# haoyu94/RoITr

Hardware: AMD Instinct MI355X
Metric: point-cloud pairs/s (higher is better)
Workload: dtype f32

## Files before the change

roitr_amd/csrc/local_block.hip:

```cpp
#include "common.h"
#include "prof.h"
#include "roitr_engine.h"
#include <mutex>
#include <vector>

namespace {

typedef float f32x4 __attribute__((ext_vector_type(4)));
typedef float f32x16 __attribute__((ext_vector_type(16)));
typedef float f32x2 __attribute__((ext_vector_type(2)));
typedef __bf16 bf16x8 __attribute__((ext_vector_type(8)));
typedef __bf16 bf16x2 __attribute__((ext_vector_type(2)));


template <int CTRL> __device__ __forceinline__ float dpp_mov(float v)
{
    return __int_as_float(__builtin_amdgcn_update_dpp(0, __float_as_int(v), CTRL, 0xf, 0xf, true));
}
template <int HL> __device__ __forceinline__ float head_allsum(float v)
{
    v += dpp_mov<0xB1>(v);
    v += dpp_mov<0x4E>(v);
    if (HL == 8) v += dpp_mov<0x141>(v);
    return v;
}

struct Acc { f32x4 t[2][2]; };

__device__ __forceinline__ void acc_zero(Acc& a)
{
#pragma unroll
    for (int m = 0; m < 2; ++m)
#pragma unroll
        for (int n = 0; n < 2; ++n) a.t[m][n] = f32x4{0.f, 0.f, 0.f, 0.f};
}

template <int H, int AP, int RT = 1, bool FR = false, bool APF = false>
__device__ __forceinline__ void gemm_phase(Acc (&acc)[RT], const float* __restrict__ A, int Ka, const float* __restrict__ W, int ldw, int k_w0,
                                           int r0, int c0, int tid)
{
    const int lane = tid & 63, i = lane & 15, g = lane >> 4;
    const float* wl = FR ? W + ((size_t)(c0 >> 5) * (ldw >> 5) + (k_w0 >> 5)) * 1024 + 4 * lane : W + (size_t)(c0 + i) * ldw + k_w0 + 4 * g;
    const int os = FR ? 1024 : 32, oc = FR ? 512 : 16, on = FR ? 256 : 16 * ldw;
    const float* al = A + (r0 + i) * AP + 4 * g;
    float4 bn[2][2];
#pragma unroll
    for (int c = 0; c < 2; ++c) { bn[c][0] = *reinterpret_cast<const float4*>(wl + c * oc); bn[c][1] = *reinterpret_cast<const float4*>(wl + c * oc + on); }
    float4 an0, an1;
    if (APF) { an0 = *reinterpret_cast<const float4*>(al); an1 = *reinterpret_cast<const float4*>(al + 16 * AP); }
    for (int k0 = 0; k0 < Ka; k0 += 32) {
        float4 bc[2][2];
#pragma unroll
        for (int c = 0; c < 2; ++c) { bc[c][0] = bn[c][0]; bc[c][1] = bn[c][1]; }
        if (k0 + 32 < Ka) {
            const float* wn = wl + (size_t)((k0 >> 5) + 1) * os;
#pragma unroll
            for (int c = 0; c < 2; ++c) {
                bn[c][0] = *reinterpret_cast<const float4*>(wn + c * oc);
                bn[c][1] = *reinterpret_cast<const float4*>(wn + c * oc + on);
            }
        }
#pragma unroll
        for (int c = 0; c < 2; ++c) {
            const float4 b0 = bc[c][0], b1 = bc[c][1];
#pragma unroll
            for (int t = 0; t < RT; ++t) {
                float4 a0, a1;
                if (APF) {
                    a0 = an0; a1 = an1;
                    const bool last = t + 1 == RT && c == 1;
                    const int tn = t + 1 < RT ? t + 1 : 0, kn = last ? k0 + 32 : k0 + (t + 1 < RT ? 16 * c : 16);
                    if (!last || k0 + 32 < Ka) {
                        an0 = *reinterpret_cast<const float4*>(al + 32 * tn * AP + kn);
                        an1 = *reinterpret_cast<const float4*>(al + (32 * tn + 16) * AP + kn);
                    }
                    __builtin_amdgcn_sched_barrier(0);
                } else {
                    a0 = *reinterpret_cast<const float4*>(al + 32 * t * AP + k0 + 16 * c);
                    a1 = *reinterpret_cast<const float4*>(al + (32 * t + 16) * AP + k0 + 16 * c);
                }
#define LB_STEP(S)                                                                                                  \
                acc[t].t[0][0] = __builtin_amdgcn_mfma_f32_16x16x4f32(a0.S, b0.S, acc[t].t[0][0], 0, 0, 0);          \
                acc[t].t[0][1] = __builtin_amdgcn_mfma_f32_16x16x4f32(a0.S, b1.S, acc[t].t[0][1], 0, 0, 0);          \
                acc[t].t[1][0] = __builtin_amdgcn_mfma_f32_16x16x4f32(a1.S, b0.S, acc[t].t[1][0], 0, 0, 0);          \
                acc[t].t[1][1] = __builtin_amdgcn_mfma_f32_16x16x4f32(a1.S, b1.S, acc[t].t[1][1], 0, 0, 0)
                LB_STEP(x); LB_STEP(y); LB_STEP(z); LB_STEP(w);
#undef LB_STEP
            }
        }
    }
}
template <int H, int AP, bool FR = false, bool APF = false>
__device__ __forceinline__ void gemm_phase1(Acc& acc, const float* __restrict__ A, int Ka, const float* __restrict__ W, int ldw, int k_w0,
                                           int r0, int c0, int tid)
{
    gemm_phase<H, AP, 1, FR, APF>(reinterpret_cast<Acc (&)[1]>(acc), A, Ka, W, ldw, k_w0, r0, c0, tid);
}

template <int DP>
__device__ __forceinline__ void acc_store(const Acc& acc, const float* __restrict__ bias, float* __restrict__ D, int r0, int c0, int lane)
{
#pragma unroll
    for (int n = 0; n < 2; ++n) {
        const int col = c0 + 16 * n + (lane & 15);
        const float bv = bias[col];
#pragma unroll
        for (int m = 0; m < 2; ++m)
#pragma unroll
            for (int r = 0; r < 4; ++r) D[(r0 + 16 * m + 4 * (lane >> 4) + r) * DP + col] = acc.t[m][n][r] + bv;
    }
}

__device__ __forceinline__ unsigned lb_pack_bf16(float x, float y)
{
    f32x2 v = {x, y};
    return __builtin_bit_cast(unsigned, __builtin_convertvector(v, bf16x2));
}
template <int AP, int RT>
__device__ __forceinline__ void gemm_phase_bf16(f32x16 (&acc)[RT], const float* __restrict__ A, int Ka, const unsigned short* __restrict__ Wb, int ldw,
                                                int k_w0, int r0, int c0, int tid)
{
    const int lane = tid & 63, ml = lane & 31, kh = lane >> 5;
    const unsigned short* w = Wb + (size_t)(c0 + ml) * ldw + k_w0 + 8 * kh;
    uint4 bn[2];
    bn[0] = *reinterpret_cast<const uint4*>(w); bn[1] = *reinterpret_cast<const uint4*>(w + 16);
    for (int k0 = 0; k0 < Ka; k0 += 32) {
        uint4 bc[2] = {bn[0], bn[1]};
        if (k0 + 32 < Ka) { bn[0] = *reinterpret_cast<const uint4*>(w + k0 + 32); bn[1] = *reinterpret_cast<const uint4*>(w + k0 + 48); }
#pragma unroll
        for (int c = 0; c < 2; ++c) {
            const bf16x8 b = __builtin_bit_cast(bf16x8, bc[c]);
#pragma unroll
            for (int t = 0; t < RT; ++t) {
                const float* ap = A + (r0 + 32 * t + ml) * AP + k0 + 16 * c + 8 * kh;
                const float4 x0 = *reinterpret_cast<const float4*>(ap), x1 = *reinterpret_cast<const float4*>(ap + 4);
                const uint4 h = make_uint4(lb_pack_bf16(x0.x, x0.y), lb_pack_bf16(x0.z, x0.w), lb_pack_bf16(x1.x, x1.y), lb_pack_bf16(x1.z, x1.w));
                acc[t] = __builtin_amdgcn_mfma_f32_32x32x16_bf16(__builtin_bit_cast(bf16x8, h), b, acc[t], 0, 0, 0);
            }
        }
    }
}
template <int DP>
__device__ __forceinline__ void acc_store32(const f32x16& acc, const float* __restrict__ bias, float* __restrict__ D, int r0, int c0, int lane)
{
    const int col = c0 + (lane & 31);
    const float bv = bias[col];
#pragma unroll
    for (int i = 0; i < 16; ++i) D[(r0 + (i & 3) + 8 * (i >> 2) + 4 * (lane >> 5)) * DP + col] = acc[i] + bv;
}
template <bool MB, int RT> struct RegionAcc { Acc a[RT]; };
template <int RT> struct RegionAcc<true, RT> { f32x16 a[RT]; };
template <bool MB, int RT> __device__ __forceinline__ void region_zero(RegionAcc<MB, RT>& r)
{
#pragma unroll
    for (int t = 0; t < RT; ++t) {
        if constexpr (MB) {
#pragma unroll
            for (int i = 0; i < 16; ++i) r.a[t][i] = 0.f;
        } else acc_zero(r.a[t]);
    }
}
template <bool MB, int H, int AP, int RT, bool FR, bool APF>
__device__ __forceinline__ void region_gemm(RegionAcc<MB, RT>& r, const float* __restrict__ A, int Ka, const float* __restrict__ W,
                                            const unsigned short* __restrict__ Wb, int ldw, int k_w0, int r0, int c0, int tid)
{
    if constexpr (MB) gemm_phase_bf16<AP, RT>(r.a, A, Ka, Wb, ldw, k_w0, r0, c0, tid);
    else gemm_phase<H, AP, RT, FR, APF>(r.a, A, Ka, W, ldw, k_w0, r0, c0, tid);
}
template <bool MB, int DP, int RT>
__device__ __forceinline__ void region_store(const RegionAcc<MB, RT>& r, const float* __restrict__ bias, float* __restrict__ D, int r0, int c0, int lane)
{
#pragma unroll
    for (int t = 0; t < RT; ++t) {
        if constexpr (MB) acc_store32<DP>(r.a[t], bias, D, r0 + 32 * t, c0, lane);
        else acc_store<DP>(r.a[t], bias, D, r0 + 32 * t, c0, lane);
    }
}

template <bool KVH>
__device__ __forceinline__ float4 ld_kv4(const float* kv, size_t row, int ld, int col)
{
    if (KVH) {
        const uint2 t = *reinterpret_cast<const uint2*>(reinterpret_cast<const unsigned short*>(kv) + row * ld + col);
        return make_float4(__uint_as_float(t.x << 16), __uint_as_float(t.x & 0xffff0000u), __uint_as_float(t.y << 16), __uint_as_float(t.y & 0xffff0000u));
    }
    return *reinterpret_cast<const float4*>(kv + row * ld + col);
}

template <int H, int K, int TM, int DBG = 0, bool KVH = false, bool MB = false, bool FR = false>
__global__ __launch_bounds__(256, (K <= 8 && TM * H <= 4096) ? 3 : 2) void local_block_kernel(RoitrLocalBlock a)
{
    constexpr int AP = H + 4;
    constexpr int LPN = H / 4;
    constexpr int NPW = 64 / LPN;
    constexpr int HL = LPN / 4;
    constexpr int HV = H / 64;
    __shared__ __attribute__((aligned(16))) float R1[TM * AP];
    __shared__ __attribute__((aligned(16))) float R2[TM * AP];
    __shared__ int ids[TM];
    int tid = threadIdx.x, lane = tid & 63, wave = tid >> 6;
    const int ntiles = (a.M + TM - 1) / TM;
    const int tile = xcd_block_id(ntiles);
    if (tile >= ntiles) return;
    const int s0 = tile * TM;
    if (tid < TM) {
        const int sl = s0 + tid < a.M ? s0 + tid : s0;
        ids[tid] = a.node_order ? __float_as_int(reinterpret_cast<const float4*>(a.node_order)[sl].w) : sl;
    }
    __syncthreads();
    {
        constexpr int F4 = H / 4;
        constexpr int NX = TM * F4 / 256;
        float4 xr[NX];
#pragma unroll
        for (int u = 0; u < NX; ++u) {
            const int e = tid + 256 * u;
            xr[u] = *reinterpret_cast<const float4*>(a.x + (size_t)ids[e / F4] * H + 4 * (e % F4));
        }
#pragma unroll
        for (int u = 0; u < NX; ++u) {
            const int e = tid + 256 * u;
            *reinterpret_cast<float4*>(R1 + (e / F4) * AP + 4 * (e % F4)) = xr[u];
        }
    }
    constexpr int NC = H / 32, RT = TM * H / (32 * 32 * 4);
    constexpr bool APF = H == 128 && RT == 2;
    int r0 = (wave / NC) * 32 * RT;
    int c0 = (wave % NC) * 32;
    RegionAcc<MB, RT> acc;
    auto zero_all = [&]() { region_zero<MB, RT>(acc); };
    auto store_all = [&](const float* bias) { region_store<MB, AP, RT>(acc, bias, R2, r0, c0, lane); };
    __syncthreads();
    zero_all();
    if (DBG != 2) region_gemm<MB, H, AP, RT, FR, APF>(acc, R1, H, a.wq, a.wq_h, H, 0, r0, c0, tid);
    store_all(a.bq);
    __syncthreads();
    if (DBG != 1) {
        const int ns = lane / LPN, j = lane % LPN, jq = j % HL;
        const int t4 = jq & 3;
        constexpr int NRD = TM / (4 * NPW);
        int gi[K]; float pv[K];
        auto load_ids = [&](int rd_, int (&g_)[K], float (&p_)[K]) {
            const int node_ = ids[(rd_ * 4 + wave) * NPW + ns];
            const int4* gp = reinterpret_cast<const int4*>(a.group_idx + (size_t)node_ * K);
#pragma unroll
            for (int q4 = 0; q4 < K / 4; ++q4) { const int4 t = gp[q4]; g_[4 * q4] = t.x; g_[4 * q4 + 1] = t.y; g_[4 * q4 + 2] = t.z; g_[4 * q4 + 3] = t.w; }
            const float* pf = a.ppf + (size_t)node_ * K * 4 + t4;
#pragma unroll
            for (int kk = 0; kk < K; ++kk) p_[kk] = pf[kk * 4];
        };
        load_ids(0, gi, pv);
        for (int rd = 0; rd < NRD; ++rd) {
            const int row = (rd * 4 + wave) * NPW + ns;
            constexpr bool V_EARLY = K <= 8;
            float4 kr[K], vr[K];
#pragma unroll
            for (int kk = 0; kk < K; ++kk) kr[kk] = ld_kv4<KVH>(a.kv, (size_t)gi[kk], 2 * H, 4 * j);
            if (V_EARLY) {
#pragma unroll
                for (int kk = 0; kk < K; ++kk) vr[kk] = ld_kv4<KVH>(a.kv, (size_t)gi[kk], 2 * H, H + 4 * j);
            }
            int gn[K]; float pn[K];
            if (rd + 1 < NRD) load_ids(rd + 1, gn, pn);
            float4 wpe4[4]; float bpe4[4];
#pragma unroll
            for (int i = 0; i < 4; ++i) { wpe4[i] = reinterpret_cast<const float4*>(a.wpe)[4 * j + i]; bpe4[i] = a.bpe[4 * j + i]; }
            float4 qv = *reinterpret_cast<const float4*>(R2 + row * AP + 4 * j);
            float ec, c4;
            {
                float p0 = 0.f, p1 = 0.f, p2 = 0.f, p3 = 0.f, p4 = 0.f;
                const float qs[4] = {qv.x, qv.y, qv.z, qv.w};
#pragma unroll
                for (int i = 0; i < 4; ++i) {
                    p0 = fmaf(wpe4[i].x, qs[i], p0); p1 = fmaf(wpe4[i].y, qs[i], p1); p2 = fmaf(wpe4[i].z, qs[i], p2);
                    p3 = fmaf(wpe4[i].w, qs[i], p3); p4 = fmaf(bpe4[i], qs[i], p4);
                }
                p0 = head_allsum<HL>(p0); p1 = head_allsum<HL>(p1); p2 = head_allsum<HL>(p2); p3 = head_allsum<HL>(p3); p4 = head_allsum<HL>(p4);
                ec = jq < 4 ? (jq == 0 ? p0 : (jq == 1 ? p1 : (jq == 2 ? p2 : p3))) * a.scale : 0.f;
                c4 = jq == 0 ? p4 * a.scale : 0.f;
            }
            qv.x *= a.scale; qv.y *= a.scale; qv.z *= a.scale; qv.w *= a.scale;
            float sc[K];
            float mx = -INFINITY;
#pragma unroll
            for (int kk = 0; kk < K; ++kk) {
                float d = fmaf(ec, pv[kk], c4);
                d = fmaf(qv.x, kr[kk].x, d); d = fmaf(qv.y, kr[kk].y, d); d = fmaf(qv.z, kr[kk].z, d); d = fmaf(qv.w, kr[kk].w, d);
                d = head_allsum<HL>(d);
                sc[kk] = d;
                mx = fmaxf(mx, d);
            }
            if (!V_EARLY) {
#pragma unroll
                for (int kk = 0; kk < K; ++kk) vr[kk] = ld_kv4<KVH>(a.kv, (size_t)gi[kk], 2 * H, H + 4 * j);
            }
            float sum = 0.f;
#pragma unroll
            for (int kk = 0; kk < K; ++kk) { sc[kk] = __expf(sc[kk] - mx); sum += sc[kk]; }
            float pb = 0.f;
            float4 o = make_float4(0.f, 0.f, 0.f, 0.f);
            const float inv = 1.0f / sum;
#pragma unroll
            for (int kk = 0; kk < K; ++kk) {
                const float p = sc[kk] * inv;
                pb = fmaf(p, pv[kk], pb);
                o.x = fmaf(p, vr[kk].x, o.x); o.y = fmaf(p, vr[kk].y, o.y); o.z = fmaf(p, vr[kk].z, o.z); o.w = fmaf(p, vr[kk].w, o.w);
            }
            const float b0 = dpp_mov<0x00>(pb), b1 = dpp_mov<0x55>(pb), b2 = dpp_mov<0xAA>(pb), b3 = dpp_mov<0xFF>(pb);
            const float4 bias = *reinterpret_cast<const float4*>(a.bvpe + 4 * j);
            const float4 w0 = reinterpret_cast<const float4*>(a.wvpe)[4 * j], w1 = reinterpret_cast<const float4*>(a.wvpe)[4 * j + 1];
            const float4 w2 = reinterpret_cast<const float4*>(a.wvpe)[4 * j + 2], w3 = reinterpret_cast<const float4*>(a.wvpe)[4 * j + 3];
            o.x += w0.x * b0 + w0.y * b1 + w0.z * b2 + w0.w * b3 + bias.x;
            o.y += w1.x * b0 + w1.y * b1 + w1.z * b2 + w1.w * b3 + bias.y;
            o.z += w2.x * b0 + w2.y * b1 + w2.z * b2 + w2.w * b3 + bias.z;
            o.w += w3.x * b0 + w3.y * b1 + w3.z * b2 + w3.w * b3 + bias.w;
            *reinterpret_cast<float4*>(R2 + row * AP + 4 * j) = o;
            if (rd + 1 < NRD) {
#pragma unroll
                for (int kk = 0; kk < K; ++kk) { gi[kk] = gn[kk]; pv[kk] = pn[kk]; }
            }
        }
    }
    {
        int t2 = tid;
        asm volatile("" : "+v"(t2));
        tid = t2; lane = t2 & 63; wave = t2 >> 6;
        r0 = (wave / NC) * 32 * RT; c0 = (wave % NC) * 32;
    }
    __syncthreads();
    zero_all();
    if (DBG != 2) {
    region_gemm<MB, H, AP, RT, FR, APF>(acc, R2, H, a.wcat, a.wcat_h, 2 * H, 0, r0, c0, tid);
    region_gemm<MB, H, AP, RT, FR, APF>(acc, R1, H, a.wcat, a.wcat_h, 2 * H, H, r0, c0, tid);
    }
    __syncthreads();
    store_all(a.bcat);
    __syncthreads();
    {
        const int lr = lane >> 4, lc = lane & 15;
        float4 gam[HV], bet[HV];
#pragma unroll
        for (int i = 0; i < HV; ++i) { gam[i] = reinterpret_cast<const float4*>(a.norm_w)[lc + 16 * i]; bet[i] = reinterpret_cast<const float4*>(a.norm_b)[lc + 16 * i]; }
#pragma unroll
        for (int u = 0; u < TM / 16; ++u) {
            const int rl = (u * 4 + wave) * 4 + lr;
            float4 t[HV];
            float s_ = 0.f;
#pragma unroll
            for (int i = 0; i < HV; ++i) { t[i] = *reinterpret_cast<const float4*>(R2 + rl * AP + 4 * (lc + 16 * i)); s_ += (t[i].x + t[i].y) + (t[i].z + t[i].w); }
            const float mean = row_allsum(s_) / (float)H;
            float q_ = 0.f;
#pragma unroll
            for (int i = 0; i < HV; ++i) {
                const float dx = t[i].x - mean, dy = t[i].y - mean, dz = t[i].z - mean, dw = t[i].w - mean;
                q_ += (dx * dx + dy * dy) + (dz * dz + dw * dw);
            }
            const float rstd = 1.0f / sqrtf(row_allsum(q_) / (float)H + a.eps);
#pragma unroll
            for (int i = 0; i < HV; ++i) {
                float4 y;
                y.x = (t[i].x - mean) * rstd * gam[i].x + bet[i].x; y.y = (t[i].y - mean) * rstd * gam[i].y + bet[i].y;
                y.z = (t[i].z - mean) * rstd * gam[i].z + bet[i].z; y.w = (t[i].w - mean) * rstd * gam[i].w + bet[i].w;
                *reinterpret_cast<float4*>(R1 + rl * AP + 4 * (lc + 16 * i)) = y;
            }
        }
    }
    float4 xres[TM / 16][HV];
    {
        const int lr = lane >> 4, lc = lane & 15;
#pragma unroll
        for (int u = 0; u < TM / 16; ++u) {
            const size_t node = (size_t)ids[(u * 4 + wave) * 4 + lr];
#pragma unroll
            for (int i = 0; i < HV; ++i) xres[u][i] = *reinterpret_cast<const float4*>(a.x + node * H + 4 * (lc + 16 * i));
        }
    }
    __syncthreads();
    zero_all();
    if (DBG != 2) region_gemm<MB, H, AP, RT, FR, APF>(acc, R1, H, a.wout, a.wout_h, H, 0, r0, c0, tid);
    __syncthreads();
    store_all(a.bout);
    __syncthreads();
    {
        const int lr = lane >> 4, lc = lane & 15;
        float4 gam[HV], bet[HV];
#pragma unroll
        for (int i = 0; i < HV; ++i) { gam[i] = reinterpret_cast<const float4*>(a.bn2_w)[lc + 16 * i]; bet[i] = reinterpret_cast<const float4*>(a.bn2_b)[lc + 16 * i]; }
#pragma unroll
        for (int u = 0; u < TM / 16; ++u) {
            const int rl = (u * 4 + wave) * 4 + lr;
            float4 t[HV];
            float s_ = 0.f;
#pragma unroll
            for (int i = 0; i < HV; ++i) { t[i] = *reinterpret_cast<const float4*>(R2 + rl * AP + 4 * (lc + 16 * i)); s_ += (t[i].x + t[i].y) + (t[i].z + t[i].w); }
            const float mean = row_allsum(s_) / (float)H;
            float q_ = 0.f;
#pragma unroll
            for (int i = 0; i < HV; ++i) {
                const float dx = t[i].x - mean, dy = t[i].y - mean, dz = t[i].z - mean, dw = t[i].w - mean;
                q_ += (dx * dx + dy * dy) + (dz * dz + dw * dw);
            }
            const float rstd = 1.0f / sqrtf(row_allsum(q_) / (float)H + a.eps);
            if (s0 + rl < a.M) {
                const size_t node = (size_t)ids[rl];
#pragma unroll
                for (int i = 0; i < HV; ++i) {
                    float4 y;
                    y.x = fmaxf((t[i].x - mean) * rstd * gam[i].x + bet[i].x + xres[u][i].x, 0.f);
                    y.y = fmaxf((t[i].y - mean) * rstd * gam[i].y + bet[i].y + xres[u][i].y, 0.f);
                    y.z = fmaxf((t[i].z - mean) * rstd * gam[i].z + bet[i].z + xres[u][i].z, 0.f);
                    y.w = fmaxf((t[i].w - mean) * rstd * gam[i].w + bet[i].w + xres[u][i].w, 0.f);
                    *reinterpret_cast<float4*>(a.out + node * H + 4 * (lc + 16 * i)) = y;
                }
            }
        }
    }
}


template <int K, bool FR>
__global__ __launch_bounds__(256) void local_first_kernel(RoitrLocalFirst a)
{
    constexpr int H = 64, TM = 64, AP = H + 4, HV = 1;
    __shared__ __attribute__((aligned(16))) float R1[TM * AP];
    __shared__ __attribute__((aligned(16))) float R2[TM * AP];
    __shared__ int ids[TM];
    const int tid = threadIdx.x, lane = tid & 63, wave = tid >> 6;
    const int ntiles = (a.M + TM - 1) / TM;
    const int tile = xcd_block_id(ntiles);
    if (tile >= ntiles) return;
    const int s0 = tile * TM;
    if (tid < TM) {
        const int sl = s0 + tid < a.M ? s0 + tid : s0;
        ids[tid] = a.node_order ? __float_as_int(reinterpret_cast<const float4*>(a.node_order)[sl].w) : sl;
    }
    __syncthreads();
    {
        const int row = tid >> 2, h = tid & 3;
        const int node = ids[row];
        const float xi = a.x[node];
        int gi[K];
        const int4* gp = reinterpret_cast<const int4*>(a.group_idx + (size_t)node * K);
#pragma unroll
        for (int q4 = 0; q4 < K / 4; ++q4) { const int4 t = gp[q4]; gi[4 * q4] = t.x; gi[4 * q4 + 1] = t.y; gi[4 * q4 + 2] = t.z; gi[4 * q4 + 3] = t.w; }
        float4 pf[K]; float xj[K];
#pragma unroll
        for (int kk = 0; kk < K; ++kk) { pf[kk] = reinterpret_cast<const float4*>(a.ppf)[(size_t)node * K + kk]; xj[kk] = a.x[gi[kk]]; }
        const float* hc = a.head_consts + h * 16;
        const float c1 = hc[0], c2 = hc[1], c3 = hc[2], c4 = hc[3], d1 = hc[12], d0 = hc[13];
        const float p0 = fmaf(xi, hc[4], hc[8]), p1 = fmaf(xi, hc[5], hc[9]), p2 = fmaf(xi, hc[6], hc[10]), p3 = fmaf(xi, hc[7], hc[11]);
        const float base = fmaf(xi, c2 + d1, c4 + d0), slope = fmaf(xi, c1, c3);
        float sc[K];
        float mx = -INFINITY;
#pragma unroll
        for (int kk = 0; kk < K; ++kk) {
            float d = fmaf(slope, xj[kk], base);
            d = fmaf(p0, pf[kk].x, d); d = fmaf(p1, pf[kk].y, d); d = fmaf(p2, pf[kk].z, d); d = fmaf(p3, pf[kk].w, d);
            sc[kk] = d * a.scale;
            mx = fmaxf(mx, sc[kk]);
        }
        float sum = 0.f;
#pragma unroll
        for (int kk = 0; kk < K; ++kk) { sc[kk] = __expf(sc[kk] - mx); sum += sc[kk]; }
        const float inv = 1.0f / sum;
        float S = 0.f;
        float4 pb = make_float4(0.f, 0.f, 0.f, 0.f);
#pragma unroll
        for (int kk = 0; kk < K; ++kk) {
            const float p = sc[kk] * inv;
            S = fmaf(p, xj[kk], S);
            pb.x = fmaf(p, pf[kk].x, pb.x); pb.y = fmaf(p, pf[kk].y, pb.y); pb.z = fmaf(p, pf[kk].z, pb.z); pb.w = fmaf(p, pf[kk].w, pb.w);
        }
        float* g = R2 + row * AP;
        g[h] = S;
        *reinterpret_cast<float4*>(g + 4 + 4 * h) = pb;
        if (h == 0) {
            g[20] = xi; g[21] = 1.0f;
            *reinterpret_cast<float2*>(g + 22) = make_float2(0.f, 0.f);
            *reinterpret_cast<float4*>(g + 24) = make_float4(0.f, 0.f, 0.f, 0.f);
            *reinterpret_cast<float4*>(g + 28) = make_float4(0.f, 0.f, 0.f, 0.f);
        }
    }
    const int r0 = (wave >> 1) * 32, c0 = (wave & 1) * 32;
    Acc acc;
    __syncthreads();
    acc_zero(acc);
    gemm_phase1<H, AP, false, false>(acc, R2, 32, a.G, 32, 0, r0, c0, tid);
    __syncthreads();
    acc_store<AP>(acc, a.zero_bias, R2, r0, c0, lane);
    __syncthreads();
    {
        const int lr = lane >> 4, lc = lane & 15;
        const float4 gam = reinterpret_cast<const float4*>(a.norm_w)[lc], bet = reinterpret_cast<const float4*>(a.norm_b)[lc];
#pragma unroll
        for (int u = 0; u < TM / 16; ++u) {
            const int rl = (u * 4 + wave) * 4 + lr;
            const float4 t = *reinterpret_cast<const float4*>(R2 + rl * AP + 4 * lc);
            const float mean = row_allsum((t.x + t.y) + (t.z + t.w)) / (float)H;
            const float dx = t.x - mean, dy = t.y - mean, dz = t.z - mean, dw = t.w - mean;
            const float rstd = 1.0f / sqrtf(row_allsum((dx * dx + dy * dy) + (dz * dz + dw * dw)) / (float)H + a.eps);
            float4 y;
            y.x = dx * rstd * gam.x + bet.x; y.y = dy * rstd * gam.y + bet.y; y.z = dz * rstd * gam.z + bet.z; y.w = dw * rstd * gam.w + bet.w;
            *reinterpret_cast<float4*>(R1 + rl * AP + 4 * lc) = y;
        }
    }
    __syncthreads();
    acc_zero(acc);
    gemm_phase1<H, AP, FR, false>(acc, R1, H, a.wout, H, 0, r0, c0, tid);
    __syncthreads();
    acc_store<AP>(acc, a.bout, R2, r0, c0, lane);
    __syncthreads();
    {
        const int lr = lane >> 4, lc = lane & 15;
#pragma unroll
        for (int u = 0; u < TM / 16; ++u) {
            const int rl = (u * 4 + wave) * 4 + lr;
            if (s0 + rl < a.M)
                *reinterpret_cast<float4*>(a.out + (size_t)ids[rl] * H + 4 * lc) = *reinterpret_cast<const float4*>(R2 + rl * AP + 4 * lc);
        }
    }
    (void)HV;
}


template <int HQ> struct TdVec;
template <> struct TdVec<2> {
    static __device__ __forceinline__ void ld(const float* p, float (&v)[2]) { const float2 t = *reinterpret_cast<const float2*>(p); v[0] = t.x; v[1] = t.y; }
    static __device__ __forceinline__ void st(float* p, const float (&v)[2]) { *reinterpret_cast<float2*>(p) = make_float2(v[0], v[1]); }
};
__device__ __forceinline__ float td_row_allmax(float v)
{
    v = fmaxf(v, dpp_get<0xB1>(v)); v = fmaxf(v, dpp_get<0x4E>(v)); v = fmaxf(v, dpp_get<0x141>(v)); v = fmaxf(v, dpp_get<0x140>(v));
    return v;
}

template <bool FR>
__global__ __launch_bounds__(256, 3) void local_td_kernel(RoitrLocalTd a)
{
    constexpr int I = 64, H = 128, K = 16, TM = 32, HQ = 2, HV = 2;
    constexpr int P2 = H + 4, P3 = 4 * I + 4;
    __shared__ __attribute__((aligned(16))) float R2[TM * P2];
    __shared__ __attribute__((aligned(16))) float R3[TM * P3];
    __shared__ __attribute__((aligned(16))) float probs[4][64];
    __shared__ int ids[TM];
    const int tid = threadIdx.x, lane = tid & 63, wave = tid >> 6;
    const int ntiles = (a.M + TM - 1) / TM;
    const int tile = xcd_block_id(ntiles);
    if (tile >= ntiles) return;
    const int s0 = tile * TM;
    if (tid < TM) {
        const int sl = s0 + tid < a.M ? s0 + tid : s0;
        ids[tid] = a.node_order ? __float_as_int(reinterpret_cast<const float4*>(a.node_order)[sl].w) : sl;
    }
    __syncthreads();
    {
        constexpr int F4 = I / 4, NX = TM * F4 / 256;
        float4 xr[NX];
#pragma unroll
        for (int u = 0; u < NX; ++u) {
            const int e = tid + 256 * u;
            xr[u] = *reinterpret_cast<const float4*>(a.x + (size_t)a.node_idx[ids[e / F4]] * I + 4 * (e % F4));
        }
#pragma unroll
        for (int u = 0; u < NX; ++u) {
            const int e = tid + 256 * u;
            *reinterpret_cast<float4*>(R2 + (e / F4) * P2 + 4 * (e % F4)) = xr[u];
        }
    }
    __syncthreads();
    const int c0 = wave * 32;
    {
        Acc accq;
#pragma unroll
        for (int pass = 0; pass < 3; ++pass) {
            Acc acc;
            acc_zero(acc);
            gemm_phase1<H, P2, FR, true>(acc, R2, I, a.wqqt, I, 0, 0, 128 * pass + c0, tid);
            if (pass == 0) accq = acc;
            else {
#pragma unroll
                for (int n = 0; n < 2; ++n) {
                    const int col = 128 * (pass - 1) + c0 + 16 * n + (lane & 15);
                    const float bv = a.bqqt[H + col];
#pragma unroll
                    for (int m = 0; m < 2; ++m)
#pragma unroll
                        for (int r = 0; r < 4; ++r) R3[(16 * m + 4 * (lane >> 4) + r) * P3 + col] = acc.t[m][n][r] + bv;
                }
            }
        }
        __syncthreads();
        acc_store<P2>(accq, a.bqqt, R2, 0, c0, lane);
    }
    __syncthreads();
    {
        const int h = lane >> 4, i16 = lane & 15, kk_l = row16_slot(i16);
        float4 wpe2[HQ]; float bvpe2[HQ]; float4 wvpe2[HQ];
#pragma unroll
        for (int i = 0; i < HQ; ++i) {
            wpe2[i] = reinterpret_cast<const float4*>(a.wpe)[lane * HQ + i];
            wvpe2[i] = reinterpret_cast<const float4*>(a.wvpe)[lane * HQ + i];
            bvpe2[i] = a.bvpe[lane * HQ + i];
        }
        constexpr int NPB = TM / 4;
        int g_cur = a.group_idx[(size_t)ids[wave * NPB] * K + i16];
        float4 pf_cur = reinterpret_cast<const float4*>(a.ppf)[(size_t)ids[wave * NPB] * K + kk_l];
        int g_nx = a.group_idx[(size_t)ids[wave * NPB + 1] * K + i16];
        float4 pf_nx = reinterpret_cast<const float4*>(a.ppf)[(size_t)ids[wave * NPB + 1] * K + kk_l];
        float xr[K], xn[K];
#pragma unroll
        for (int kk = 0; kk < K; ++kk) xr[kk] = a.x[(size_t)__builtin_amdgcn_readlane(g_cur, kk) * I + lane];
        for (int nn = 0; nn < NPB; ++nn) {
            const int row = wave * NPB + nn;
            const float4 pf = pf_cur;
            if (nn + 1 < NPB) {
#pragma unroll
                for (int kk = 0; kk < K; ++kk) xn[kk] = a.x[(size_t)__builtin_amdgcn_readlane(g_nx, kk) * I + lane];
            }
            int g_n2 = 0; float4 pf_n2 = make_float4(0.f, 0.f, 0.f, 0.f);
            if (nn + 2 < NPB) {
                g_n2 = a.group_idx[(size_t)ids[row + 2] * K + i16];
                pf_n2 = reinterpret_cast<const float4*>(a.ppf)[(size_t)ids[row + 2] * K + kk_l];
            }
            float qt[4], qv[HQ];
#pragma unroll
            for (int hh = 0; hh < 4; ++hh) qt[hh] = R3[row * P3 + hh * I + lane];
            TdVec<HQ>::ld(R2 + row * P2 + lane * HQ, qv);
            float u0 = 0.f, u1 = 0.f, u2 = 0.f, u3 = 0.f;
#pragma unroll
            for (int i = 0; i < HQ; ++i) {
                u0 = fmaf(wpe2[i].x, qv[i], u0); u1 = fmaf(wpe2[i].y, qv[i], u1); u2 = fmaf(wpe2[i].z, qv[i], u2); u3 = fmaf(wpe2[i].w, qv[i], u3);
            }
            u0 = row_allsum(u0); u1 = row_allsum(u1); u2 = row_allsum(u2); u3 = row_allsum(u3);
            float z[16];
            {
                float w[32];
#pragma unroll
                for (int i = 0; i < 32; ++i) {
                    const int h0 = i >> 4, k0 = i & 15;
                    w[i] = swap32_sum(qt[h0] * xr[k0], qt[h0 + 2] * xr[k0]);
                }
#pragma unroll
                for (int i = 0; i < 16; ++i) z[i] = swap16_sum(w[i], w[i + 16]);
            }
            const float tot = row16_transpose_sum(z, lane);
            const float s = (tot + (u0 * pf.x + u1 * pf.y + u2 * pf.z + u3 * pf.w)) * a.scale;
            const float mx = td_row_allmax(s);
            const float e = expf(s - mx);
            const float p = e / row_allsum(e);
            probs[wave][h * 16 + kk_l] = p;
            const float pb0 = row_allsum(p * pf.x), pb1 = row_allsum(p * pf.y), pb2 = row_allsum(p * pf.z), pb3 = row_allsum(p * pf.w);
            {
                float o[HQ];
#pragma unroll
                for (int i = 0; i < HQ; ++i) o[i] = wvpe2[i].x * pb0 + wvpe2[i].y * pb1 + wvpe2[i].z * pb2 + wvpe2[i].w * pb3 + bvpe2[i];
                TdVec<HQ>::st(R2 + row * P2 + lane * HQ, o);
            }
            asm volatile("s_waitcnt lgkmcnt(0)" ::: "memory");
#pragma unroll
            for (int hh = 0; hh < 4; ++hh) {
                float acc = 0.f;
#pragma unroll
                for (int q4 = 0; q4 < 4; ++q4) {
                    const float4 p4 = reinterpret_cast<const float4*>(probs[wave])[hh * 4 + q4];
                    acc = fmaf(p4.x, xr[4 * q4], acc); acc = fmaf(p4.y, xr[4 * q4 + 1], acc);
                    acc = fmaf(p4.z, xr[4 * q4 + 2], acc); acc = fmaf(p4.w, xr[4 * q4 + 3], acc);
                }
                R3[row * P3 + hh * I + lane] = acc;
            }
            asm volatile("s_waitcnt lgkmcnt(0)" ::: "memory");
#pragma unroll
            for (int kk = 0; kk < K; ++kk) xr[kk] = xn[kk];
            pf_cur = pf_nx; g_nx = g_n2; pf_nx = pf_n2;
        }
    }
    __syncthreads();
    {
        Acc acc;
        acc_zero(acc);
        gemm_phase1<H, P3, FR, true>(acc, R3 + I * wave, I, a.wv, I, 0, 0, c0, tid);
#pragma unroll
        for (int n = 0; n < 2; ++n) {
            const int col = c0 + 16 * n + (lane & 15);
            const float bv = a.bv[col];
#pragma unroll
            for (int m = 0; m < 2; ++m)
#pragma unroll
                for (int r = 0; r < 4; ++r) {
                    float* d = R2 + (16 * m + 4 * (lane >> 4) + r) * P2 + col;
                    *d = *d + (acc.t[m][n][r] + bv);
                }
        }
    }
    constexpr int F4n = I / 4;
    int e0 = tid, e1 = tid + 256;
    asm volatile("" : "+v"(e0), "+v"(e1));
    const float4 xn_a = *reinterpret_cast<const float4*>(a.x + (size_t)a.node_idx[ids[e0 / F4n]] * I + 4 * (e0 % F4n));
    const float4 xn_b = *reinterpret_cast<const float4*>(a.x + (size_t)a.node_idx[ids[e1 / F4n]] * I + 4 * (e1 % F4n));
    __syncthreads();
    *reinterpret_cast<float4*>(R3 + (e0 / F4n) * P3 + 2 * I + 4 * (e0 % F4n)) = xn_a;
    *reinterpret_cast<float4*>(R3 + (e1 / F4n) * P3 + 2 * I + 4 * (e1 % F4n)) = xn_b;
    Acc acc;
    acc_zero(acc);
    gemm_phase1<H, P2, FR, true>(acc, R2, H, a.wcat, H + I, 0, 0, c0, tid);
    __syncthreads();
    gemm_phase1<H, P3, FR, true>(acc, R3 + 2 * I, I, a.wcat, H + I, H, 0, c0, tid);
    acc_store<P2>(acc, a.bcat, R2, 0, c0, lane);
    __syncthreads();
    {
        const int lr = lane >> 4, lc = lane & 15;
        float4 gam[HV], bet[HV];
#pragma unroll
        for (int i = 0; i < HV; ++i) { gam[i] = reinterpret_cast<const float4*>(a.norm_w)[lc + 16 * i]; bet[i] = reinterpret_cast<const float4*>(a.norm_b)[lc + 16 * i]; }
#pragma unroll
        for (int u = 0; u < TM / 16; ++u) {
            const int rl = (u * 4 + wave) * 4 + lr;
            float4 t[HV];
            float s_ = 0.f;
#pragma unroll
            for (int i = 0; i < HV; ++i) { t[i] = *reinterpret_cast<const float4*>(R2 + rl * P2 + 4 * (lc + 16 * i)); s_ += (t[i].x + t[i].y) + (t[i].z + t[i].w); }
            const float mean = row_allsum(s_) / (float)H;
            float q_ = 0.f;
#pragma unroll
            for (int i = 0; i < HV; ++i) {
                const float dx = t[i].x - mean, dy = t[i].y - mean, dz = t[i].z - mean, dw = t[i].w - mean;
                q_ += (dx * dx + dy * dy) + (dz * dz + dw * dw);
            }
            const float rstd = 1.0f / sqrtf(row_allsum(q_) / (float)H + a.eps);
#pragma unroll
            for (int i = 0; i < HV; ++i) {
                float4 y;
                y.x = (t[i].x - mean) * rstd * gam[i].x + bet[i].x; y.y = (t[i].y - mean) * rstd * gam[i].y + bet[i].y;
                y.z = (t[i].z - mean) * rstd * gam[i].z + bet[i].z; y.w = (t[i].w - mean) * rstd * gam[i].w + bet[i].w;
                *reinterpret_cast<float4*>(R3 + rl * P3 + 4 * (lc + 16 * i)) = y;
            }
        }
    }
    __syncthreads();
    acc_zero(acc);
    gemm_phase1<H, P3, FR, true>(acc, R3, H, a.wout, H, 0, 0, c0, tid);
    acc_store<P2>(acc, a.bout, R2, 0, c0, lane);
    __syncthreads();
    {
        const int lr = lane >> 4, lc = lane & 15;
#pragma unroll
        for (int u = 0; u < TM / 16; ++u) {
            const int rl = (u * 4 + wave) * 4 + lr;
            if (s0 + rl < a.M) {
#pragma unroll
                for (int i = 0; i < HV; ++i)
                    *reinterpret_cast<float4*>(a.out + (size_t)ids[rl] * H + 4 * (lc + 16 * i)) = *reinterpret_cast<const float4*>(R2 + rl * P2 + 4 * (lc + 16 * i));
            }
        }
    }
}

__host__ __device__ inline size_t lb_frag_src(size_t d, int k, int ldw)
{
    const int lane = (int)(d & 63), q = (int)((d >> 6) & 3), nslab = k >> 5;
    const size_t blk = d >> 8, region = blk / nslab, slab = blk % nslab;
    const int i = lane & 15, g = lane >> 4, c = q >> 1, n = q & 1;
    return (32 * region + 16 * n + i) * (size_t)ldw + 32 * slab + 16 * c + 4 * g;
}
__global__ __launch_bounds__(256) void lb_reorder_kernel(const float* __restrict__ W, int rows, int k, int ldw, float4* __restrict__ dst)
{
    const size_t d = (size_t)blockIdx.x * 256 + threadIdx.x;
    if (d < (size_t)rows * k / 4) dst[d] = *reinterpret_cast<const float4*>(W + lb_frag_src(d, k, ldw));
}
bool lb_frag_shape_ok(int rows, int k, int ldw) { return rows > 0 && k > 0 && rows % 32 == 0 && k % 32 == 0 && ldw >= k && ldw % 4 == 0; }

struct FragEntry { const float* W; int rows, k, ldw; float* frag; };
std::mutex g_frag_mutex;
std::vector<FragEntry> g_frags;

const float* lb_frag(const float* W, int rows, int k, int ldw)
{
    std::lock_guard<std::mutex> lock(g_frag_mutex);
    for (const FragEntry& e : g_frags)
        if (e.W == W && e.rows == rows && e.k == k && e.ldw == ldw) return e.frag;
    return nullptr;
}

}

extern "C" int roitr_local_weights_reorder_host(const float* src, int rows, int k, int ldw, float* dst)
{
    if (!src || !dst || !lb_frag_shape_ok(rows, k, ldw)) { roitr_set_error("roitr_local_weights_reorder_host: rows and k multiples of 32, ldw >= k", __FILE__, __LINE__); return ROITR_ERR_ARG; }
    const size_t n4 = (size_t)rows * k / 4;
    for (size_t d = 0; d < n4; ++d) { const float* s4 = src + lb_frag_src(d, k, ldw); for (int e = 0; e < 4; ++e) dst[4 * d + e] = s4[e]; }
    return ROITR_OK;
}

extern "C" int roitr_local_weights_prepare(const float* W, int rows, int k, int ldw, hipStream_t stream)
{
    if (!W || ((uintptr_t)W & 15) != 0 || !lb_frag_shape_ok(rows, k, ldw)) {
        roitr_set_error("roitr_local_weights_prepare: W 16-byte aligned, rows and k multiples of 32, ldw >= k and a multiple of 4", __FILE__, __LINE__);
        return ROITR_ERR_ARG;
    }
    float* frag = nullptr;
    {
        std::lock_guard<std::mutex> lock(g_frag_mutex);
        for (const FragEntry& e : g_frags)
            if (e.W == W && e.rows == rows && e.k == k && e.ldw == ldw) frag = e.frag;
        if (!frag) {
            ROITR_HIP(hipMalloc((void**)&frag, sizeof(float) * (size_t)rows * k));
            g_frags.push_back(FragEntry{W, rows, k, ldw, frag});
        }
    }
    lb_reorder_kernel<<<div_up(rows * k / 4, 256), 256, 0, stream>>>(W, rows, k, ldw, reinterpret_cast<float4*>(frag));
    ROITR_LAUNCH_CHECK();
    return ROITR_OK;
}

extern "C" int roitr_local_weights_count(void)
{
    std::lock_guard<std::mutex> lock(g_frag_mutex);
    return (int)g_frags.size();
}

extern "C" int roitr_local_weights_release(const float* W)
{
    std::vector<float*> drop;
    {
        std::lock_guard<std::mutex> lock(g_frag_mutex);
        for (size_t j = 0; j < g_frags.size();) {
            if (g_frags[j].W == W) { drop.push_back(g_frags[j].frag); g_frags.erase(g_frags.begin() + j); }
            else ++j;
        }
    }
    for (float* f : drop) ROITR_HIP(hipFree(f));
    return ROITR_OK;
}

extern "C" int roitr_local_block_supported(int H, int K)
{
    return ((H == 64 && K == 8) || (H == 64 && K == 16) || (H == 128 && K == 16) || (H == 128 && K == 8)) ? 1 : 0;
}

static bool lb_block_fragments(RoitrLocalBlock& b)
{
    if (b.wq_h || b.kv_bf16) return false;
    const float* wq = lb_frag(b.wq, b.H, b.H, b.H);
    const float* wcat = lb_frag(b.wcat, b.H, 2 * b.H, 2 * b.H);
    const float* wout = lb_frag(b.wout, b.H, b.H, b.H);
    if (!wq || !wcat || !wout) return false;
    b.wq = wq; b.wcat = wcat; b.wout = wout;
    return true;
}

extern "C" int roitr_local_block_dbg(const RoitrLocalBlock* a, int variant, hipStream_t stream)
{
    if (a->M <= 0 || !roitr_local_block_supported(a->H, a->K)) return ROITR_ERR_UNSUPPORTED;
    const int big = variant / 10, ph = variant % 10;
    const int tm = (a->H == 64 ? 64 : 32) * (big ? 2 : 1);
    const int grid = xcd_grid(div_up(a->M, tm));
    RoitrLocalBlock b = *a;
    const bool fr = lb_block_fragments(b);
#define LB_DBG_(HH, KK, TT, FR_)                                                                                    \
    do {                                                                                                            \
        if (ph == 1) local_block_kernel<HH, KK, TT, 1, false, false, FR_><<<grid, 256, 0, stream>>>(b);             \
        else if (ph == 2) local_block_kernel<HH, KK, TT, 2, false, false, FR_><<<grid, 256, 0, stream>>>(b);        \
        else local_block_kernel<HH, KK, TT, 0, false, false, FR_><<<grid, 256, 0, stream>>>(b);                     \
    } while (0)
#define LB_DBG(HH, KK, TT) do { if (fr) LB_DBG_(HH, KK, TT, true); else LB_DBG_(HH, KK, TT, false); } while (0)
    if (a->H == 64 && a->K == 8) { if (big) LB_DBG(64, 8, 128); else LB_DBG(64, 8, 64); }
    else if (a->H == 128 && a->K == 16) { if (big) LB_DBG(128, 16, 64); else LB_DBG(128, 16, 32); }
    else return ROITR_ERR_UNSUPPORTED;
#undef LB_DBG
#undef LB_DBG_
    ROITR_LAUNCH_CHECK();
    return ROITR_OK;
}

extern "C" int roitr_local_block(const RoitrLocalBlock* a, hipStream_t stream)
{
    if (a->M <= 0) return ROITR_OK;
    if (!roitr_local_block_supported(a->H, a->K)) return ROITR_ERR_UNSUPPORTED;
    if ((((uintptr_t)a->x | (uintptr_t)a->kv | (uintptr_t)a->group_idx | (uintptr_t)a->ppf | (uintptr_t)a->out | (uintptr_t)a->wq | (uintptr_t)a->wcat |
          (uintptr_t)a->wout | (uintptr_t)a->wpe | (uintptr_t)a->wvpe | (uintptr_t)a->bvpe | (uintptr_t)a->norm_w | (uintptr_t)a->norm_b |
          (uintptr_t)a->bn2_w | (uintptr_t)a->bn2_b) & 15) != 0) {
        roitr_set_error("roitr_local_block: operands must be 16-byte aligned", __FILE__, __LINE__);
        return ROITR_ERR_ARG;
    }
    const bool mb = a->wq_h || a->wcat_h || a->wout_h;
    if (mb && (!a->wq_h || !a->wcat_h || !a->wout_h || !a->kv_bf16 || (((uintptr_t)a->wq_h | (uintptr_t)a->wcat_h | (uintptr_t)a->wout_h) & 15) != 0)) {
        roitr_set_error("roitr_local_block: wq_h / wcat_h / wout_h go together (16-byte aligned) and with kv_bf16", __FILE__, __LINE__);
        return ROITR_ERR_ARG;
    }
    const double H = a->H, K = a->K;
    roitr_prof_begin2(ROITR_PROF_LOCAL_BLOCK, (double)a->M * (2.0 * H * 4 + K * (2.0 * H * (a->kv_bf16 ? 2 : 4) + 20.0)), 2.0 * a->M * H * H * 4.0, stream);
    constexpr int LB_BIG_MIN_TILES = 1024;
    const bool big = a->H == 128 && div_up(a->M, 64) >= LB_BIG_MIN_TILES;
    const int grid = xcd_grid(div_up(a->M, a->H == 64 ? 64 : (big ? 64 : 32)));
    RoitrLocalBlock b = *a;
    const bool fr = lb_block_fragments(b);
#define LB_GO(HH, KK, TT, KVH_) local_block_kernel<HH, KK, TT, 0, KVH_><<<grid, 256, 0, stream>>>(b)
#define LB_GO_MB(HH, KK, TT) local_block_kernel<HH, KK, TT, 0, true, true><<<grid, 256, 0, stream>>>(b)
#define LB_PICK(HH, KK, TT)                                   \
    do {                                                      \
        if (mb) LB_GO_MB(HH, KK, TT);                         \
        else if (a->kv_bf16) LB_GO(HH, KK, TT, true);         \
        else if (fr) local_block_kernel<HH, KK, TT, 0, false, false, true><<<grid, 256, 0, stream>>>(b); \
        else LB_GO(HH, KK, TT, false);                        \
    } while (0)
    if (a->H == 64) { if (a->K == 8) LB_PICK(64, 8, 64); else LB_PICK(64, 16, 64); }
    else if (big) { if (a->K == 8) LB_PICK(128, 8, 64); else LB_PICK(128, 16, 64); }
    else { if (a->K == 8) LB_PICK(128, 8, 32); else LB_PICK(128, 16, 32); }
#undef LB_PICK
#undef LB_GO_MB
#undef LB_GO
    roitr_prof_end(ROITR_PROF_LOCAL_BLOCK, stream);
    ROITR_LAUNCH_CHECK();
    return ROITR_OK;
}

extern "C" int roitr_local_td_supported(int in_dim, int H, int K) { return in_dim == 64 && H == 128 && K == 16 ? 1 : 0; }

extern "C" int roitr_local_td(const RoitrLocalTd* a, hipStream_t stream)
{
    if (a->M <= 0) return ROITR_OK;
    if (!roitr_local_td_supported(a->in_dim, a->H, 16)) return ROITR_ERR_UNSUPPORTED;
    if ((((uintptr_t)a->x | (uintptr_t)a->group_idx | (uintptr_t)a->ppf | (uintptr_t)a->out | (uintptr_t)a->wqqt | (uintptr_t)a->wv | (uintptr_t)a->wcat |
          (uintptr_t)a->wout | (uintptr_t)a->wpe | (uintptr_t)a->wvpe | (uintptr_t)a->bvpe | (uintptr_t)a->norm_w | (uintptr_t)a->norm_b) & 15) != 0 ||
        !a->node_idx || !a->bqqt || !a->bv || !a->bcat || !a->bout) {
        roitr_set_error("roitr_local_td: operands must be given and 16-byte aligned", __FILE__, __LINE__);
        return ROITR_ERR_ARG;
    }
    const double I = a->in_dim, H = a->H;
    roitr_prof_begin2(ROITR_PROF_LOCAL_BLOCK, (double)a->M * (I * 4 + 16.0 * (I * 4 + 20.0) + H * 4), 2.0 * a->M * ((H + 4 * I) * I + H * I + H * (H + I) + H * H), stream);
    RoitrLocalTd b = *a;
    {
        const int Hi = a->H, Ii = a->in_dim;
        const float* wqqt = lb_frag(b.wqqt, Hi + 4 * Ii, Ii, Ii);
        const float* wv = lb_frag(b.wv, Hi, Ii, Ii);
        const float* wcat = lb_frag(b.wcat, Hi, Hi + Ii, Hi + Ii);
        const float* wout = lb_frag(b.wout, Hi, Hi, Hi);
        if (wqqt && wv && wcat && wout) {
            b.wqqt = wqqt; b.wv = wv; b.wcat = wcat; b.wout = wout;
            local_td_kernel<true><<<xcd_grid(div_up(a->M, 32)), 256, 0, stream>>>(b);
        } else local_td_kernel<false><<<xcd_grid(div_up(a->M, 32)), 256, 0, stream>>>(b);
    }
    roitr_prof_end(ROITR_PROF_LOCAL_BLOCK, stream);
    ROITR_LAUNCH_CHECK();
    return ROITR_OK;
}

extern "C" int roitr_local_first(const RoitrLocalFirst* a, hipStream_t stream)
{
    if (a->M <= 0) return ROITR_OK;
    if (a->K != 8 && a->K != 16) return ROITR_ERR_UNSUPPORTED;
    if ((((uintptr_t)a->group_idx | (uintptr_t)a->ppf | (uintptr_t)a->out | (uintptr_t)a->G | (uintptr_t)a->wout | (uintptr_t)a->norm_w |
          (uintptr_t)a->norm_b | (uintptr_t)a->head_consts) & 15) != 0) {
        roitr_set_error("roitr_local_first: operands must be 16-byte aligned", __FILE__, __LINE__);
        return ROITR_ERR_ARG;
    }
    roitr_prof_begin2(ROITR_PROF_LOCAL_BLOCK, (double)a->M * (4.0 + a->K * (4.0 + 4.0 + 16.0) + 64.0 * 4), 2.0 * a->M * 64.0 * (32.0 + 64.0), stream);
    const int grid = xcd_grid(div_up(a->M, 64));
    RoitrLocalFirst b = *a;
    const float* wout = lb_frag(b.wout, 64, 64, 64);
    if (wout) {
        b.wout = wout;
        if (a->K == 8) local_first_kernel<8, true><<<grid, 256, 0, stream>>>(b);
        else local_first_kernel<16, true><<<grid, 256, 0, stream>>>(b);
    } else {
        if (a->K == 8) local_first_kernel<8, false><<<grid, 256, 0, stream>>>(b);
        else local_first_kernel<16, false><<<grid, 256, 0, stream>>>(b);
    }
    roitr_prof_end(ROITR_PROF_LOCAL_BLOCK, stream);
    ROITR_LAUNCH_CHECK();
    return ROITR_OK;
}
```

Before: 6639.

## Coalesce local_first neighbor feature gathers through shared memory and merge LDS buffers

Changes the first local block kernel so the block loads PPF features cooperatively in a coalesced pattern. Each of the four lanes per row now gathers only a quarter of the neighbor x values, and both are staged in LDS before each lane reads its row. The two 64x68 shared buffers are merged into one, and launch bounds now request higher occupancy (8 or 4 blocks per CU). A debug entry point with phase-isolation variants is also added. This adds a barrier and LDS traffic, and may raise register pressure under the tighter launch bounds.

```diff
diff --git a/roitr_amd/csrc/local_block.hip b/roitr_amd/csrc/local_block.hip
--- a/roitr_amd/csrc/local_block.hip
+++ b/roitr_amd/csrc/local_block.hip
@@ -418,34 +418,87 @@
 }
 
 
-template <int K, bool FR>
-__global__ __launch_bounds__(256) void local_first_kernel(RoitrLocalFirst a)
+template <int K, bool FR, int DBG = 0, bool COOP = true>
+__global__ __launch_bounds__(256, K == 8 ? 8 : 4) void local_first_kernel(RoitrLocalFirst a)
 {
     constexpr int H = 64, TM = 64, AP = H + 4, HV = 1;
-    __shared__ __attribute__((aligned(16))) float R1[TM * AP];
-    __shared__ __attribute__((aligned(16))) float R2[TM * AP];
+    constexpr int PP = K + 1;
+    constexpr int KQ = K / 4;
+    constexpr bool PF_IN_R = COOP && 32 + 4 * K <= H;
+    __shared__ __attribute__((aligned(16))) float R[TM * AP];
+    __shared__ __attribute__((aligned(16))) float PFR[COOP && !PF_IN_R ? TM * PP * 4 : 4];
+    __shared__ __attribute__((aligned(16))) float XJ[COOP ? TM * K : 4];
     __shared__ int ids[TM];
+    auto pf_at = [&](int slot, int kk) { return PF_IN_R ? reinterpret_cast<float4*>(R + slot * AP + 32) + kk : reinterpret_cast<float4*>(PFR) + slot * PP + kk; };
     const int tid = threadIdx.x, lane = tid & 63, wave = tid >> 6;
     const int ntiles = (a.M + TM - 1) / TM;
     const int tile = xcd_block_id(ntiles);
     if (tile >= ntiles) return;
     const int s0 = tile * TM;
-    if (tid < TM) {
-        const int sl = s0 + tid < a.M ? s0 + tid : s0;
-        ids[tid] = a.node_order ? __float_as_int(reinterpret_cast<const float4*>(a.node_order)[sl].w) : sl;
-    }
-    __syncthreads();
+    const int r0 = (wave >> 1) * 32, c0 = (wave & 1) * 32;
+    auto slot_node = [&](int slot) {
+        const int sl = s0 + slot < a.M ? s0 + slot : s0;
+        return a.node_order ? __float_as_int(reinterpret_cast<const float*>(a.node_order)[4 * (size_t)sl + 3]) : sl;
+    };
+    if constexpr (!COOP) {
+        if (tid < TM) ids[tid] = slot_node(tid);
+        __syncthreads();
+    }
     {
         const int row = tid >> 2, h = tid & 3;
-        const int node = ids[row];
-        const float xi = a.x[node];
-        int gi[K];
-        const int4* gp = reinterpret_cast<const int4*>(a.group_idx + (size_t)node * K);
-#pragma unroll
-        for (int q4 = 0; q4 < K / 4; ++q4) { const int4 t = gp[q4]; gi[4 * q4] = t.x; gi[4 * q4 + 1] = t.y; gi[4 * q4 + 2] = t.z; gi[4 * q4 + 3] = t.w; }
+        float xi, S;
+        float4 pb;
+        int node;
+        if constexpr (DBG == 2) {
+            node = slot_node(row);
+            if (COOP && h == 0) ids[row] = node;
+            xi = 1.0f; S = 0.25f * (float)h; pb = make_float4(0.01f * (float)row, 0.5f, -0.5f, 0.125f * (float)h);
+        } else {
         float4 pf[K]; float xj[K];
-#pragma unroll
-        for (int kk = 0; kk < K; ++kk) { pf[kk] = reinterpret_cast<const float4*>(a.ppf)[(size_t)node * K + kk]; xj[kk] = a.x[gi[kk]]; }
+        if constexpr (COOP) {
+            constexpr int NP = TM * K / 256;
+            node = slot_node(row);
+            int pn[NP];
+#pragma unroll
+            for (int j = 0; j < NP; ++j) pn[j] = slot_node((j * 256 + tid) / K);
+            float4 pp[NP];
+#pragma unroll
+            for (int j = 0; j < NP; ++j) pp[j] = reinterpret_cast<const float4*>(a.ppf)[(size_t)pn[j] * K + (j * 256 + tid) % K];
+            int gq[KQ];
+            const int* gp = a.group_idx + (size_t)node * K + KQ * h;
+            if constexpr (K == 8) { const int2 t = *reinterpret_cast<const int2*>(gp); gq[0] = t.x; gq[1] = t.y; }
+            else { const int4 t = *reinterpret_cast<const int4*>(gp); gq[0] = t.x; gq[1] = t.y; gq[2] = t.z; gq[3] = t.w; }
+            xi = a.x[node];
+            float xq[KQ];
+#pragma unroll
+            for (int j = 0; j < KQ; ++j) xq[j] = a.x[gq[j]];
+            if (h == 0) ids[row] = node;
+#pragma unroll
+            for (int j = 0; j < NP; ++j) {
+                const int p = j * 256 + tid;
+                *pf_at(p / K, p % K) = pp[j];
+            }
+            float* xs = XJ + row * K + KQ * h;
+            if constexpr (K == 8) *reinterpret_cast<float2*>(xs) = make_float2(xq[0], xq[1]);
+            else *reinterpret_cast<float4*>(xs) = make_float4(xq[0], xq[1], xq[2], xq[3]);
+            __syncthreads();
+#pragma unroll
+            for (int kk = 0; kk < K; ++kk) pf[kk] = *pf_at(row, kk);
+#pragma unroll
+            for (int q4 = 0; q4 < KQ; ++q4) {
+                const float4 t = *reinterpret_cast<const float4*>(XJ + row * K + 4 * q4);
+                xj[4 * q4] = t.x; xj[4 * q4 + 1] = t.y; xj[4 * q4 + 2] = t.z; xj[4 * q4 + 3] = t.w;
+            }
+        } else {
+            node = ids[row];
+            xi = a.x[node];
+            int gi[K];
+            const int4* gp = reinterpret_cast<const int4*>(a.group_idx + (size_t)node * K);
+#pragma unroll
+            for (int q4 = 0; q4 < K / 4; ++q4) { const int4 t = gp[q4]; gi[4 * q4] = t.x; gi[4 * q4 + 1] = t.y; gi[4 * q4 + 2] = t.z; gi[4 * q4 + 3] = t.w; }
+#pragma unroll
+            for (int kk = 0; kk < K; ++kk) { pf[kk] = reinterpret_cast<const float4*>(a.ppf)[(size_t)node * K + kk]; xj[kk] = a.x[gi[kk]]; }
+        }
         const float* hc = a.head_consts + h * 16;
         const float c1 = hc[0], c2 = hc[1], c3 = hc[2], c4 = hc[3], d1 = hc[12], d0 = hc[13];
         const float p0 = fmaf(xi, hc[4], hc[8]), p1 = fmaf(xi, hc[5], hc[9]), p2 = fmaf(xi, hc[6], hc[10]), p3 = fmaf(xi, hc[7], hc[11]);
@@ -463,15 +516,20 @@
 #pragma unroll
         for (int kk = 0; kk < K; ++kk) { sc[kk] = __expf(sc[kk] - mx); sum += sc[kk]; }
         const float inv = 1.0f / sum;
-        float S = 0.f;
-        float4 pb = make_float4(0.f, 0.f, 0.f, 0.f);
+        S = 0.f;
+        pb = make_float4(0.f, 0.f, 0.f, 0.f);
 #pragma unroll
         for (int kk = 0; kk < K; ++kk) {
             const float p = sc[kk] * inv;
             S = fmaf(p, xj[kk], S);
             pb.x = fmaf(p, pf[kk].x, pb.x); pb.y = fmaf(p, pf[kk].y, pb.y); pb.z = fmaf(p, pf[kk].z, pb.z); pb.w = fmaf(p, pf[kk].w, pb.w);
         }
-        float* g = R2 + row * AP;
+        }
+        if constexpr (DBG == 1) {
+            if (s0 + row < a.M) a.out[(size_t)node * H + h] = S + ((pb.x + pb.y) + (pb.z + pb.w)) + xi;
+            return;
+        }
+        float* g = R + row * AP;
         g[h] = S;
         *reinterpret_cast<float4*>(g + 4 + 4 * h) = pb;
         if (h == 0) {
@@ -481,13 +539,12 @@
             *reinterpret_cast<float4*>(g + 28) = make_float4(0.f, 0.f, 0.f, 0.f);
         }
     }
-    const int r0 = (wave >> 1) * 32, c0 = (wave & 1) * 32;
     Acc acc;
     __syncthreads();
     acc_zero(acc);
-    gemm_phase1<H, AP, false, false>(acc, R2, 32, a.G, 32, 0, r0, c0, tid);
-    __syncthreads();
-    acc_store<AP>(acc, a.zero_bias, R2, r0, c0, lane);
+    gemm_phase1<H, AP, false, false>(acc, R, 32, a.G, 32, 0, r0, c0, tid);
+    __syncthreads();
+    acc_store<AP>(acc, a.zero_bias, R, r0, c0, lane);
     __syncthreads();
     {
         const int lr = lane >> 4, lc = lane & 15;
@@ -495,20 +552,20 @@
 #pragma unroll
         for (int u = 0; u < TM / 16; ++u) {
             const int rl = (u * 4 + wave) * 4 + lr;
-            const float4 t = *reinterpret_cast<const float4*>(R2 + rl * AP + 4 * lc);
+            const float4 t = *reinterpret_cast<const float4*>(R + rl * AP + 4 * lc);
             const float mean = row_allsum((t.x + t.y) + (t.z + t.w)) / (float)H;
             const float dx = t.x - mean, dy = t.y - mean, dz = t.z - mean, dw = t.w - mean;
             const float rstd = 1.0f / sqrtf(row_allsum((dx * dx + dy * dy) + (dz * dz + dw * dw)) / (float)H + a.eps);
             float4 y;
             y.x = dx * rstd * gam.x + bet.x; y.y = dy * rstd * gam.y + bet.y; y.z = dz * rstd * gam.z + bet.z; y.w = dw * rstd * gam.w + bet.w;
-            *reinterpret_cast<float4*>(R1 + rl * AP + 4 * lc) = y;
+            *reinterpret_cast<float4*>(R + rl * AP + 4 * lc) = y;
         }
     }
     __syncthreads();
     acc_zero(acc);
-    gemm_phase1<H, AP, FR, false>(acc, R1, H, a.wout, H, 0, r0, c0, tid);
-    __syncthreads();
-    acc_store<AP>(acc, a.bout, R2, r0, c0, lane);
+    gemm_phase1<H, AP, FR, false>(acc, R, H, a.wout, H, 0, r0, c0, tid);
+    __syncthreads();
+    acc_store<AP>(acc, a.bout, R, r0, c0, lane);
     __syncthreads();
     {
         const int lr = lane >> 4, lc = lane & 15;
@@ -516,7 +573,7 @@
         for (int u = 0; u < TM / 16; ++u) {
             const int rl = (u * 4 + wave) * 4 + lr;
             if (s0 + rl < a.M)
-                *reinterpret_cast<float4*>(a.out + (size_t)ids[rl] * H + 4 * lc) = *reinterpret_cast<const float4*>(R2 + rl * AP + 4 * lc);
+                *reinterpret_cast<float4*>(a.out + (size_t)ids[rl] * H + 4 * lc) = *reinterpret_cast<const float4*>(R + rl * AP + 4 * lc);
         }
     }
     (void)HV;
@@ -945,8 +1002,9 @@
     return ROITR_OK;
 }
 
-extern "C" int roitr_local_first(const RoitrLocalFirst* a, hipStream_t stream)
-{
+static int lf_check(const RoitrLocalFirst* a, bool* go)
+{
+    *go = false;
     if (a->M <= 0) return ROITR_OK;
     if (a->K != 8 && a->K != 16) return ROITR_ERR_UNSUPPORTED;
     if ((((uintptr_t)a->group_idx | (uintptr_t)a->ppf | (uintptr_t)a->out | (uintptr_t)a->G | (uintptr_t)a->wout | (uintptr_t)a->norm_w |
@@ -954,6 +1012,41 @@
         roitr_set_error("roitr_local_first: operands must be 16-byte aligned", __FILE__, __LINE__);
         return ROITR_ERR_ARG;
     }
+    *go = true;
+    return ROITR_OK;
+}
+
+extern "C" int roitr_local_first_dbg(const RoitrLocalFirst* a, int variant, hipStream_t stream)
+{
+    bool go;
+    const int rc = lf_check(a, &go);
+    if (rc != ROITR_OK || !go) return rc;
+    const int form = variant / 10, ph = variant % 10;
+    if (form < 0 || form > 1 || ph < 0 || ph > 2) return ROITR_ERR_ARG;
+    const int grid = xcd_grid(div_up(a->M, 64));
+    RoitrLocalFirst b = *a;
+    const float* wout = lb_frag(b.wout, 64, 64, 64);
+    if (wout) b.wout = wout;
+#define LF_PH(KK, FR_, COOP_)                                                                       \
+    do {                                                                                            \
+        if (ph == 1) local_first_kernel<KK, FR_, 1, COOP_><<<grid, 256, 0, stream>>>(b);            \
+        else if (ph == 2) local_first_kernel<KK, FR_, 2, COOP_><<<grid, 256, 0, stream>>>(b);       \
+        else local_first_kernel<KK, FR_, 0, COOP_><<<grid, 256, 0, stream>>>(b);                    \
+    } while (0)
+#define LF_FORM(KK, FR_) do { if (form == 1) LF_PH(KK, FR_, false); else LF_PH(KK, FR_, true); } while (0)
+    if (a->K == 8) { if (wout) LF_FORM(8, true); else LF_FORM(8, false); }
+    else { if (wout) LF_FORM(16, true); else LF_FORM(16, false); }
+#undef LF_FORM
+#undef LF_PH
+    ROITR_LAUNCH_CHECK();
+    return ROITR_OK;
+}
+
+extern "C" int roitr_local_first(const RoitrLocalFirst* a, hipStream_t stream)
+{
+    bool go;
+    const int rc = lf_check(a, &go);
+    if (rc != ROITR_OK || !go) return rc;
     roitr_prof_begin2(ROITR_PROF_LOCAL_BLOCK, (double)a->M * (4.0 + a->K * (4.0 + 4.0 + 16.0) + 64.0 * 4), 2.0 * a->M * 64.0 * (32.0 + 64.0), stream);
     const int grid = xcd_grid(div_up(a->M, 64));
     RoitrLocalFirst b = *a;
```

After: 6561. 0.988x the previous value.
